# tachitachi/SR-WaveNet

Measured on AMD Instinct MI355X. Metric: audio samples/sec (fwd+bwd) 30-layer teacher WaveNet, higher is better.
Workload: dtype bf16; 1 GPU; 30-layer teacher WaveNet (3x[1..512] dilations, 64 res / 256 skip ch, 256-way mu-law softmax), fwd+bwd+Adam, batch 8x16000 samples per GPU; global_batch=8, seq_len=16000, parallelism=dp1, launch=hipGraph

## Files before the change

### sr-wavenet_amd/build.py

```python
from __future__ import annotations

import os
import subprocess
import sys
from concurrent.futures import ThreadPoolExecutor

HERE = os.path.dirname(os.path.abspath(__file__))
CSRC = os.path.join(HERE, "csrc")
LIB = os.path.join(HERE, "libsrwn.so")
MANIFEST = os.path.join(HERE, "libsrwn.manifest.json")
IO_LIB = os.path.join(HERE, "libsrwn_io.so")
PYB_SRC = os.path.join(CSRC, "srwn_pybind.cpp")
PYB_NAME = "_srwn_pyb"
IO_SOURCES = ["srwn_tfrecord.cpp"]
CXX = os.environ.get("CXX", "g++")
SOURCES = ["srwn_util.hip", "srwn_fwd.hip", "srwn_bwd.hip", "srwn_opt.hip", "srwn_pool.hip", "srwn_gemm.hip", "srwn_wgrad2.hip", "srwn_gen.hip", "srwn_gen16.hip", "srwn_flow.hip", "srwn_enc.hip", "srwn_nc.hip", "srwn_ncstream.hip", "srwn_group.hip", "srwn_wgradt.hip", "srwn_ops.hip", "srwn_head.hip", "srwn_siamese.hip", "srwn_wngate.hip", "srwn_stream.hip", "srwn_recog.hip", "srwn_score.hip"]
HIPCC = os.environ.get("HIPCC", "/opt/rocm/bin/hipcc")
FLAGS = ["--offload-arch=gfx950", "-O3", "-fPIC", "-std=c++17", "-Wno-pass-failed", "-ffp-contract=on"]
NO_SPILL = {"srwn_wgradt.hip": ["wgrad_skip_wt_kernel"], "srwn_siamese.hip": ["contrastive_head_kernel"],
            "srwn_wngate.hip": ["wavenet_layer_fwd_kernel", "wavenet_layer_bwd_kernel"],
            "srwn_ncstream.hip": ["nc_encode_frames_kernel", "nc_encode_frames_kernelINS_10NcListArgs"],
            "srwn_recog.hip": ["pooled_stream_head_kernel"], "srwn_score.hip": ["stream_score_head_kernel"]}


def _deps():
    hdrs = [os.path.join(CSRC, f) for f in os.listdir(CSRC) if f.endswith(".h")]
    hdrs.append(os.path.join(HERE, "..", "include", "srwn.h"))
    return hdrs


def source_hashes():
    import hashlib
    files = [os.path.join(CSRC, f) for f in sorted(os.listdir(CSRC)) if f.endswith((".hip", ".h", ".cpp"))]
    files.append(os.path.join(HERE, "..", "include", "srwn.h"))
    files.append(os.path.join(HERE, "..", "include", "srwn_io.h"))
    out = {}
    for f in files:
        if os.path.exists(f):
            out[os.path.relpath(f, os.path.join(HERE, ".."))] = hashlib.sha256(open(f, "rb").read()).hexdigest()
    return out


def _stale(target, srcs):
    if not os.path.exists(target):
        return True
    t = os.path.getmtime(target)
    return any(os.path.getmtime(s) > t for s in srcs)


def _sha(paths, extra=""):
    import hashlib
    h = hashlib.sha256(extra.encode())
    for f in paths:
        h.update(open(f, "rb").read())
    return h.hexdigest()


def _check_no_spill(src, obj, remarks, kernels):
    import re
    seen = {}
    name = None
    for line in remarks.splitlines():
        m = re.search(r"Function Name: (\S+)", line)
        if m:
            name = m.group(1)
        m = re.search(r"(?:[VS]GPRs Spill|ScratchSize \[bytes/lane\]): (\d+)", line)
        if m and name:
            seen[name] = seen.get(name, 0) + int(m.group(1))
    for k in kernels:
        hit = [(n, v) for n, v in seen.items() if k in n]
        if not hit or any(v for _, v in hit):
            if os.path.exists(obj):
                os.remove(obj)
            raise RuntimeError("%s: kernel %s must not spill registers or use scratch: %s" % (src, k, hit or "not found"))


def _check_inflight(src, obj, flags, kernels):
    import importlib.util
    spec = importlib.util.spec_from_file_location("_srwn_asmcheck", os.path.join(HERE, "asmcheck.py"))
    ac = importlib.util.module_from_spec(spec)
    spec.loader.exec_module(ac)
    cmd = [HIPCC] + flags + ["--cuda-device-only", "-S", src, "-o", "-"]
    r = subprocess.run(cmd, capture_output=True, text=True)
    if r.returncode != 0:
        raise RuntimeError("hipcc -S failed for %s:\n%s" % (src, r.stderr[-4000:]))
    for k in kernels:
        bad = ac.check_inflight_loads(r.stdout, k)
        if bad:
            if os.path.exists(obj):
                os.remove(obj)
            raise RuntimeError("%s: kernel %s touches the destination of a load that may still be in flight:\n  %s"
                               % (src, k, "\n  ".join(bad[:8])))


def build(force: bool = False, verbose: bool = False, diag: bool = False, variant: str = "", extra_flags=()) -> str:
    import json
    per_src = {}
    for f in list(extra_flags):
        if ".hip:" in f:
            name, fl = f.split(":", 1)
            per_src.setdefault(name, []).extend(fl.split("=", 1) if fl.startswith("-mllvm=") else [fl])
    extra_flags = [f for f in extra_flags if ".hip:" not in f]
    flags = FLAGS + (["-DSRWN_DIAG"] if diag else []) + list(extra_flags)
    if variant:
        diag = True
        odir = os.path.join(CSRC, "ab_" + variant)
        os.makedirs(os.path.join(HERE, "..", "ab"), exist_ok=True)
        lib = os.path.join(HERE, "..", "ab", "libsrwn_%s.so" % variant)
    else:
        odir = os.path.join(CSRC, "diag") if diag else CSRC
        lib = os.path.join(HERE, "libsrwn_diag.so") if diag else LIB
    os.makedirs(odir, exist_ok=True)
    man_path = os.path.join(odir, "objects.manifest.json") if diag else MANIFEST
    srcs = [os.path.join(CSRC, s) for s in SOURCES if os.path.exists(os.path.join(CSRC, s))]
    objs = [os.path.join(odir, os.path.splitext(os.path.basename(s))[0] + ".o") for s in srcs]
    deps = sorted(_deps())
    try:
        old = json.load(open(man_path)).get("objects", {})
    except (OSError, ValueError):
        old = {}
    keys = {}

    def cc(pair):
        src, obj = pair
        rel = os.path.basename(src)
        sflags = flags + per_src.get(rel, [])
        key = _sha([src] + deps, " ".join(sflags))
        if force or not os.path.exists(obj) or old.get(rel) != key:
            guarded = NO_SPILL.get(rel, [])
            cmd = [HIPCC] + sflags + (["-Rpass-analysis=kernel-resource-usage"] if guarded else []) + ["-c", src, "-o", obj]
            if verbose:
                print(" ".join(cmd), flush=True)
            r = subprocess.run(cmd, capture_output=True, text=True)
            if r.returncode != 0:
                raise RuntimeError("hipcc failed for %s:\n%s" % (src, r.stderr[-8000:]))
            if guarded:
                _check_no_spill(src, obj, r.stderr, guarded)
                _check_inflight(src, obj, sflags, guarded)
        keys[rel] = key
        return obj

    with ThreadPoolExecutor(max_workers=4) as ex:
        list(ex.map(cc, zip(srcs, objs)))
    relink = force or not os.path.exists(lib) or old != keys
    if relink:
        cmd = [HIPCC, "--offload-arch=gfx950", "-shared", "-fPIC", "-o", lib] + objs
        r = subprocess.run(cmd, capture_output=True, text=True)
        if r.returncode != 0:
            raise RuntimeError("link failed:\n%s" % r.stderr[-8000:])
    if diag:
        with open(man_path, "w") as f:
            json.dump({"flags": flags, "objects": keys}, f, indent=1, sort_keys=True)
        return lib
    build_io(force)
    build_pybind(force or relink)
    with open(MANIFEST, "w") as f:
        json.dump({"flags": flags, "objects": keys, "sources": source_hashes()}, f, indent=1, sort_keys=True)
    return lib


def _signatures():
    import importlib.util
    spec = importlib.util.spec_from_file_location("_srwn_lib_for_build", os.path.join(HERE, "_lib.py"))
    m = importlib.util.module_from_spec(spec)
    spec.loader.exec_module(m)
    return m


def pybind_source() -> str:
    import ctypes as C
    L = _signatures()
# ... 66 lines not shown
```

### sr-wavenet_amd/csrc/srwn_group.h

```cpp
#pragma once
#include <cstdint>
#include <cstdlib>
#include "srwn_common.h"

namespace srwn {
namespace grp {

constexpr int kMaxGroup = 8;
constexpr int kLdsBudget = 160 * 1024;

template <typename T> struct Raw4g;
template <> struct Raw4g<bf16_t> {
  typedef bf16x4 type;
  static __device__ __forceinline__ type load(const bf16_t* p) { return *reinterpret_cast<const bf16x4*>(p); }
  static __device__ __forceinline__ float get(const type& v, int e) { return (float)v[e]; }
  static __device__ __forceinline__ type zero() { return type{(bf16_t)0.0f, (bf16_t)0.0f, (bf16_t)0.0f, (bf16_t)0.0f}; }
  static __device__ __forceinline__ type pack(float a, float b, float c, float d) {
    return type{(bf16_t)a, (bf16_t)b, (bf16_t)c, (bf16_t)d};
  }
};
template <> struct Raw4g<float> {
  typedef f32x4 type;
  static __device__ __forceinline__ type load(const float* p) { return *reinterpret_cast<const f32x4*>(p); }
  static __device__ __forceinline__ float get(const type& v, int e) { return v[e]; }
  static __device__ __forceinline__ type zero() { return type{0.f, 0.f, 0.f, 0.f}; }
  static __device__ __forceinline__ type pack(float a, float b, float c, float d) { return type{a, b, c, d}; }
};

__device__ __forceinline__ void glds16_untracked(const void* g, unsigned lds_addr) {
  unsigned keep;
  asm volatile("s_mov_b32 %0, m0\n\ts_mov_b32 m0, %2\n\ts_nop 0\n\tglobal_load_lds_dwordx4 %1, off\n\ts_mov_b32 m0, %0"
               : "=&s"(keep) : "v"(g), "s"(lds_addr) : "memory");
}
__device__ __forceinline__ void dma_wait() { asm volatile("s_waitcnt vmcnt(0)" ::: "memory"); }
__device__ __forceinline__ void dma_image(const void* gsrc, unsigned lds_dst, int nbytes, int wave, int lane,
                                          int nwaves = 8) {
  const char* g = reinterpret_cast<const char*>(gsrc) + lane * 16;
  for (int p = wave; p < nbytes / 1024; p += nwaves) glds16_untracked(g + (size_t)p * 1024, __builtin_amdgcn_readfirstlane(lds_dst + p * 1024));
}

__device__ __forceinline__ void wg_barrier() { asm volatile("s_waitcnt lgkmcnt(0)\n\ts_barrier" ::: "memory"); }

__device__ __forceinline__ constexpr int kordW(int kg, int j) { return 16 * (kg >> 1) + 2 * (kg & 1) + (j >> 2) + 4 * (j & 3); }

template <typename T> struct LdT16;
template <> struct LdT16<bf16_t> {
  static __device__ __forceinline__ Frag<bf16_t> load(const bf16_t* tile, int stride, int row0, int col0, int lane) {
    typedef short s16x4 __attribute__((ext_vector_type(4)));
    const int kg = lane >> 4, i = lane & 15, q = i >> 2, p = i & 3;
    const bf16_t* base = tile + (size_t)(row0 + 16 * (kg >> 1) + 2 * (kg & 1) + 4 * q) * stride + col0 + 4 * p;
    s16x4 lo = __builtin_amdgcn_ds_read_tr16_b64_v4i16((__attribute__((address_space(3))) s16x4*)(base));
    s16x4 hi = __builtin_amdgcn_ds_read_tr16_b64_v4i16((__attribute__((address_space(3))) s16x4*)(base + stride));
    Frag<bf16_t> f;
    f.v = __builtin_bit_cast(bf16x8, __builtin_shufflevector(lo, hi, 0, 1, 2, 3, 4, 5, 6, 7));
    return f;
  }
};
template <> struct LdT16<float> {
  static __device__ __forceinline__ Frag<float> load(const float* tile, int stride, int row0, int col0, int lane) {
    const int kg = lane >> 4;
    const float* base = tile + (size_t)row0 * stride + col0 + (lane & 15);
    Frag<float> f;
#pragma unroll
    for (int j = 0; j < 8; ++j) f.set(j, base[(size_t)kordW(kg, j) * stride]);
// ... 138 lines not shown
```

### sr-wavenet_amd/csrc/srwn_group.hip

```cpp
#include <cmath>
#include <cstdlib>
#include <type_traits>
#include <vector>
#include "srwn_common.h"
#include "srwn_group.h"
#include "srwn_host.h"
#include "../../include/srwn.h"

using namespace srwn;
using namespace srwn::grp;

namespace {

struct GroupFwdArgs {
  int safe_wait;
  const void* x0;
  void* x_out;
  void* z_out;
  int64_t layer_stride;
  const void* wconv[kMaxGroup];
  const void* wres[kMaxGroup];
  const float* bias_f[kMaxGroup];
  const float* bias_r[kMaxGroup];
  const void* cond[kMaxGroup];
// ... 478 lines not shown
      stamp(18);
    }
  }
}

struct GroupBwdArgs {
  const void* g_top;
  void* g_out;
  void* df_out;
  const void* z;
  const void* dcs;
  int64_t layer_stride;
  const void* wconvT[kMaxGroup];
  const void* wresT[kMaxGroup];
  int sub[kMaxGroup];
  int hb[kMaxGroup];
  int nl, st, Tlen, B;
  int W, H, NT, nsub, nseg;
  const void* xT; const void* cT; int64_t wt_stride; int KT;
  void* part_f; void* part_r; float* part_bf; float* part_br;
  int nslabs, write_all_g, part16;
  const float* ic_audio; float* ic_part; int ic_shift;
  unsigned long long* stamps;
  int dbg;
};
#ifdef SRWN_DIAG
#define WT_DBG(a) ((a).dbg)
#else
#define WT_DBG(a) 0
#endif

constexpr int kWtPadRows = 64;
constexpr bool kWtEarlyR = true;
constexpr bool kWtStagger = false;
constexpr bool kWtEarlyC = false;

template <typename T, int RT, bool DCS, int MAXT, int NWB, int NWV = 8, bool WT = false, bool STAMP = false, bool P16 = false, bool ICG = false>
__global__ __launch_bounds__(64 * NWV) void group_bwd_kernel(GroupBwdArgs a) {
  static_assert(!P16 || (WT && sizeof(T) == 2), "16-bit partial blocks: the bf16 weight-gradient-tile mode only");
  static_assert(!ICG || WT, "input conv gradient: the weight-gradient-tile mode only");
  constexpr int R = 32 * RT, K = 2, KS = R / 16;
  Stamper<STAMP> stamp{nullptr, 0};
  if (STAMP && blockIdx.x == 0 && (threadIdx.x & 63) == 0 && ((threadIdx.x >> 6) & 3) == 0) stamp.p = a.stamps + (threadIdx.x >> 8) * 512;
  stamp(1);
  constexpr int NCONV = RT * K * KS, NRES = RT * KS, NW = NCONV + NRES;
  constexpr int LS = RowStage<T>::stride(R), VEC = RowStage<T>::VEC;
  constexpr int LPR = R / VEC, RPI = 64 / LPR, NI = 32 / RPI;
  constexpr int WBYTES = NW * 64 * (int)sizeof(Frag<T>);
  constexpr int WPIECES = WBYTES / 16, CPIECES = NCONV * 64 * (int)sizeof(Frag<T>) / 16;
  constexpr int KTMAX = NWV * MAXT;
  typedef typename Raw4g<T>::type raw4;
  extern __shared__ __attribute__((aligned(16))) char smem[];
  Frag<T>* wbuf = reinterpret_cast<Frag<T>*>(smem);
  T* img = reinterpret_cast<T*>(smem + (size_t)NWB * WBYTES);

  const int tid = threadIdx.x, lane = tid & 63, wave = __builtin_amdgcn_readfirstlane(tid >> 6);
  const int col = lane & 31, half = lane >> 5;
  const int rsub = lane / LPR, piece = lane % LPR;

  const unsigned lds_base = (unsigned)(size_t)(__attribute__((address_space(3))) char*)smem;
  auto wload = [&](int g, int buf) {
    dma_image(a.wconvT[g], lds_base + buf * WBYTES, CPIECES * 16, wave, lane, NWV);
    dma_image(a.wresT[g], lds_base + buf * WBYTES + CPIECES * 16, (WPIECES - CPIECES) * 16, wave, lane, NWV);
  };
  const int ntw = (a.NT - wave + NWV - 1) / NWV;

  int sit = -1;
  for (int sblk = blockIdx.x; sblk < a.nseg; sblk += gridDim.x) {
    const int seg = xcd_segment(sblk, a.nseg);
    ++sit;
    const int per_clip = a.st * a.nsub;
// ... 36 lines not shown
#pragma unroll
        for (int gq = 0; gq < 4; ++gq)
          store4(trow + (size_t)col * LS + 32 * mt + 8 * gq + 4 * half, vals[mt][4 * gq], vals[mt][4 * gq + 1],
                 vals[mt][4 * gq + 2], vals[mt][4 * gq + 3]);
      wave_lds_order();
      if (hi > 0) {
#pragma unroll
        for (int i = 0; i < NI; ++i) {
          int rr = i * RPI + rsub;
          rr = rr < hi ? rr : hi - 1;
          const f32x4 v = *reinterpret_cast<const f32x4*>(trow + (size_t)rr * LS + piece * VEC);
          *reinterpret_cast<f32x4*>(gbase + grow(jbase + 32 * q + rr) * R + piece * VEC) = v;
        }
      }
    };

    auto tile_store_raw = [&](T* trow, T* gbase, int q, int hi, const raw4 (&vals)[RT][4]) {
      wave_lds_order();
#pragma unroll
      for (int mt = 0; mt < RT; ++mt)
#pragma unroll
        for (int gq = 0; gq < 4; ++gq)
          *reinterpret_cast<raw4*>(trow + (size_t)col * LS + 32 * mt + 8 * gq + 4 * half) = vals[mt][gq];
      wave_lds_order();
#pragma unroll
      for (int i = 0; i < NI; ++i) {
        int rr = i * RPI + rsub;
        rr = rr < hi ? rr : hi - 1;
        const f32x4 v = *reinterpret_cast<const f32x4*>(trow + (size_t)rr * LS + piece * VEC);
        *reinterpret_cast<f32x4*>(gbase + grow(jbase + 32 * q + rr) * R + piece * VEC) = v;
      }
    };

    raw4 G[MAXT][RT][4];
    Frag<T> acn[8];
    const int gtop = a.nl - 1;
    auto colsum = [&](float* pb_slab, int ntiles, bool mask) {
      if (!WT || wave >= R / 16) return;
      int lw = lane;
      asm volatile("" : "+v"(lw));
      const T* cb = LdT16p<T>::base(img, LS, lw) + 16 * wave;
      Frag<T> ones;
#pragma unroll
      for (int e = 0; e < 8; ++e) ones.set(e, 1.0f);
      f32x4 accb = {0.f, 0.f, 0.f, 0.f};
      const int kfull = Wseg >> 5;
      const int nfull = mask ? (kfull < ntiles ? kfull : ntiles) : ntiles;
      constexpr int CU = 4;
#pragma unroll 1
      for (int k0 = 0; k0 < nfull; k0 += CU) {
        Frag<T> bf[CU];
#pragma unroll
        for (int u = 0; u < CU; ++u) {
          const int k = k0 + u < nfull ? k0 + u : nfull - 1;
          bf[u] = LdT16p<T>::template load<LS>(cb + (size_t)(32 * k) * LS, 0);
        }
#pragma unroll
        for (int u = 0; u < CU; ++u) {
          if (k0 + u < nfull) mma16(accb, ones, bf[u]);
        }
      }
      if (mask && nfull < ntiles) {
        const int hik = Wseg - 32 * nfull;
        Frag<T> ok;
#pragma unroll
        for (int e = 0; e < 8; ++e) ok.set(e, kordW(lw >> 4, e) < hik ? 1.0f : 0.0f);
        const Frag<T> bfl = LdT16p<T>::template load<LS>(cb + (size_t)(32 * nfull) * LS, 0);
        mma16(accb, ok, bfl);
      }
      if (lw < 16) {
        float* pb = pb_slab + 16 * wave + lw;
        *pb = (sit > 0 ? *pb : 0.0f) + accb[0];
      }
    };
    if (WT) {
      f32x4* p = reinterpret_cast<f32x4*>(img);
      for (int i = tid; i < (a.NT * 32 + kWtPadRows) * LS * (int)sizeof(T) / 16; i += 64 * NWV) p[i] = f32x4{0.f, 0.f, 0.f, 0.f};
      wg_barrier();
    }
    wload(gtop, 0);
    f32x4 zr[NI], dr[NI];
    auto issue = [&](int g, int q) {
      rows_load(reinterpret_cast<const T*>(a.z) + (size_t)g * a.layer_stride, q, zr);
      if (DCS) rows_load(reinterpret_cast<const T*>(a.dcs) + (size_t)g * a.layer_stride, q, dr);
    };
#pragma unroll
    for (int m = 0; m < MAXT; ++m) {
      const int q = wave + NWV * m;
#pragma unroll
      for (int mt = 0; mt < RT; ++mt)
#pragma unroll
        for (int gq = 0; gq < 4; ++gq) G[m][mt][gq] = Raw4g<T>::zero();
      if (q < a.NT && a.g_top) {
        T* trow = img + (size_t)(32 * q) * LS;
        f32x4 v[NI];
        rows_load(reinterpret_cast<const T*>(a.g_top), q, v);
        rows_put(trow, v);
        acc_get(trow, G[m]);
        if (WT && !((jbase + 32 * q + col) < Jr)) {
#pragma unroll
          for (int mt = 0; mt < RT; ++mt)
#pragma unroll
            for (int gq = 0; gq < 4; ++gq) G[m][mt][gq] = Raw4g<T>::zero();
        }
      }
    }
    dma_wait();
    issue(gtop, wave < a.NT ? wave : a.NT - 1);
    wg_barrier();

    for (int n = 0; n < a.nl; ++n) {
      const int g = a.nl - 1 - n;
      const int d = a.sub[g];
      int wb = 0;
      if (NWB == 2) {
        wb = n & 1;
        if (g > 0) wload(g - 1, wb ^ 1);
      } else if (n > 0) {
        wload(g, 0); dma_wait(); wg_barrier();
      }
      const Frag<T>* lds_conv = wbuf + (size_t)wb * NW * 64;
      const Frag<T>* lds_res = lds_conv + NCONV * 64;
      T* dfg = reinterpret_cast<T*>(a.df_out) + (size_t)g * a.layer_stride;
      T* gprev = reinterpret_cast<T*>(a.g_out) + (size_t)(g + 1) * a.layer_stride;
      const bool haveg = (n > 0) || (a.g_top != nullptr);
      const int hb = a.hb[g];
      int ntA = (Wseg + hb + d + 31) / 32, ntB = (Wseg + hb + 31) / 32;
      ntA = (a.H == 0 || ntA > a.NT) ? a.NT : ntA;
      ntB = (a.H == 0 || ntB > a.NT) ? a.NT : ntB;

      constexpr int NIB = R / 16, NBLK = NIB * NIB;
      constexpr int NBW = NBLK >= NWV ? NBLK / NWV : 1;
      const bool active2 = NBLK >= NWV || wave < NBLK;
      const int blk2 = wave * NBW, ib2 = blk2 / NIB, ob2 = blk2 - ib2 * NIB;
      const size_t pslab = (size_t)g * a.nslabs + blockIdx.x;
      const int ktn = (Wseg + 31) / 32;
      if (WT) {
        const bool active = active2;
        const int ib = ib2, ob0 = ob2;
        f32x4 acc[NBW];
#pragma unroll
        for (int bb = 0; bb < NBW; ++bb) acc[bb] = f32x4{0.f, 0.f, 0.f, 0.f};
        int lw = lane;
        asm volatile("" : "+v"(lw));
        if (kWtEarlyR && sizeof(T) == 2 && haveg && active && !(WT_DBG(a) & 1)) {
          const T* ct0 = reinterpret_cast<const T*>(a.cT) + (size_t)g * a.wt_stride + (size_t)seg * a.KT * (R * 32);
#pragma unroll
          for (int j = 0; j < 8; ++j) acn[j] = wt_load(ct0 + (size_t)(j < ktn ? j : (ktn > 0 ? ktn - 1 : 0)) * (R * 32), 16 * ib, lw);
        }
        if (haveg) {
#pragma unroll
          for (int m = 0; m < MAXT; ++m) {
            const int q = wave + NWV * m;
            int hi = Wseg - 32 * q;
            hi = hi > 32 ? 32 : hi;
            if (q < a.NT && hi > 0) {
              T* trow = img + (size_t)(32 * q) * LS;
              const bool own = col < hi;
              wave_lds_order();
#pragma unroll
              for (int mt = 0; mt < RT; ++mt)
#pragma unroll
                for (int gq = 0; gq < 4; ++gq)
                  *reinterpret_cast<raw4*>(trow + (size_t)col * LS + 32 * mt + 8 * gq + 4 * half) = own ? G[m][mt][gq] : Raw4g<T>::zero();
              wave_lds_order();
              if (a.write_all_g && n > 0) {
#pragma unroll
                for (int i = 0; i < NI; ++i) {
                  int rr = i * RPI + rsub;
                  rr = rr < hi ? rr : hi - 1;
                  const f32x4 v = *reinterpret_cast<const f32x4*>(trow + (size_t)rr * LS + piece * VEC);
                  *reinterpret_cast<f32x4*>(gprev + grow(jbase + 32 * q + rr) * R + piece * VEC) = v;
                }
              }
            }
          }
          stamp(20);
          wg_barrier();
          stamp(21);
          colsum(a.part_br + pslab * R, ktn, false);
          if (active && !(WT_DBG(a) & 1)) {
            const T* ct = reinterpret_cast<const T*>(a.cT) + (size_t)g * a.wt_stride + (size_t)seg * a.KT * (R * 32);
            const T* gbase = LdT16p<T>::base(img, LS, lw) + 16 * ob0;
            Frag<T> av[8], bv[8];
            if ((kWtEarlyR && sizeof(T) == 2) || (kWtEarlyC && n > 0)) {
#pragma unroll
              for (int j = 0; j < 8; ++j) av[j] = acn[j];
            } else {
#pragma unroll
              for (int j = 0; j < 8; ++j) av[j] = wt_load(ct + (size_t)(j < ktn ? j : (ktn > 0 ? ktn - 1 : 0)) * (R * 32), 16 * ib, lw);
            }
            auto group8 = [&](int k0, Frag<T> (&cur)[8], Frag<T> (&nxt)[8]) __attribute__((always_inline)) {
#pragma unroll
              for (int j = 0; j < 8; ++j) {
                const int kn = k0 + 8 + j;
                if ((WT_DBG(a) & 128) && (wave & 1)) nxt[j] = zero_frag<T>();
                else
                nxt[j] = wt_load(ct + (size_t)(kn < ktn ? kn : ktn - 1) * (R * 32), 16 * ib, lw);
              }
#pragma unroll
              for (int j = 0; j < 8; ++j) {
                const int k = k0 + j;
// ... 35 lines not shown
              }
              if (!(WT_DBG(a) & 16)) __builtin_nontemporal_store(Raw4g<bf16_t>::pack(acc[bb][0], acc[bb][1], acc[bb][2], acc[bb][3]), reinterpret_cast<p4*>(pl + bb * 256));
            }
          } else {
          float* pl = reinterpret_cast<float*>(a.part_r) + pslab * (R * R) + (size_t)(16 * ib + 4 * (lw >> 4)) * R + 16 * ob0 + (lw & 15);
          if (sit > 0) {
#pragma unroll
            for (int bb = 0; bb < NBW; ++bb) {
#pragma unroll
              for (int rr = 0; rr < 4; ++rr) acc[bb][rr] += pl[rr * R + 16 * bb];
            }
          }
#pragma unroll
          for (int bb = 0; bb < NBW; ++bb) {
            if (!(WT_DBG(a) & 16)) {
#pragma unroll
            for (int rr = 0; rr < 4; ++rr) pl[rr * R + 16 * bb] = acc[bb][rr];
            }
          }
          }
        }
        if (!haveg) colsum(a.part_br + pslab * R, 0, false);
      }

      stamp(24);
#pragma unroll
      for (int m = 0; m < MAXT; ++m) {
        const int q = wave + NWV * m;
        if (q >= ntA) continue;
        T* trow = img + (size_t)(32 * q) * LS;
        const bool ok = (jbase + 32 * q + col) < Jr;
        int hi = Wseg - 32 * q;
        hi = hi > 32 ? 32 : hi;
        if (!WT && n > 0 && hi > 0) tile_store_raw(trow, gprev, q, hi, G[m]);
        raw4 zz[RT][4], dc0[RT][4];
        rows_put(trow, zr);
        acc_get(trow, zz);
        if (DCS) { rows_put(trow, dr); acc_get(trow, dc0); }
        {
          const bool same = (m + 1 < MAXT) && (q + NWV < ntA);
          if (same) issue(g, q + NWV);
          else if (g > 0) issue(g - 1, wave < a.NT ? wave : a.NT - 1);
        }
        f32x16 accC[RT];
        if (DCS && !ok) {
#pragma unroll
          for (int mt = 0; mt < RT; ++mt)
#pragma unroll
            for (int gq = 0; gq < 4; ++gq) dc0[mt][gq] = Raw4g<T>::zero();
        }
#pragma unroll
        for (int mt = 0; mt < RT; ++mt)
#pragma unroll
          for (int gq = 0; gq < 4; ++gq)
#pragma unroll
            for (int e = 0; e < 4; ++e) accC[mt][4 * gq + e] = DCS ? Raw4g<T>::get(dc0[mt][gq], e) : 0.0f;
        if (haveg) {
#pragma unroll
          for (int s = 0; s < KS; ++s) {
            Frag<T> bfr;
            if constexpr (WT && sizeof(T) == 2) {
              bf16x4 hv[2];
#pragma unroll
              for (int h2 = 0; h2 < 2; ++h2) {
                const raw4& gr = G[m][s >> 1][2 * (s & 1) + h2];
                f32x4 g4 = {Raw4g<T>::get(gr, 0), Raw4g<T>::get(gr, 1), Raw4g<T>::get(gr, 2), Raw4g<T>::get(gr, 3)};
                g4 = g4 * f32x4{kSqrtHalf, kSqrtHalf, kSqrtHalf, kSqrtHalf};
                hv[h2] = Raw4g<bf16_t>::pack(g4[0], g4[1], g4[2], g4[3]);
              }
              bfr.v = __builtin_shufflevector(hv[0], hv[1], 0, 1, 2, 3, 4, 5, 6, 7);
            } else
#pragma unroll
            for (int jj = 0; jj < 8; ++jj)
              bfr.set(jj, ((WT || ok) ? Raw4g<T>::get(G[m][s >> 1][2 * (s & 1) + (jj >> 2)], jj & 3) : 0.0f) * kSqrtHalf);
#pragma unroll
            for (int mt = 0; mt < RT; ++mt) mma(accC[mt], lds_res[(mt * KS + s) * 64 + lane], bfr);
          }
        }
        float dv[RT][16];
        if constexpr (sizeof(T) == 2) {
#pragma unroll
          for (int mt = 0; mt < RT; ++mt)
#pragma unroll
            for (int gq = 0; gq < 4; ++gq) {
              const f32x4 z4 = {Raw4g<T>::get(zz[mt][gq], 0), Raw4g<T>::get(zz[mt][gq], 1), Raw4g<T>::get(zz[mt][gq], 2), Raw4g<T>::get(zz[mt][gq], 3)};
              const f32x4 a4 = {accC[mt][4 * gq], accC[mt][4 * gq + 1], accC[mt][4 * gq + 2], accC[mt][4 * gq + 3]};
              const f32x4 d4 = a4 * dgate_df4(z4);
#pragma unroll
              for (int e = 0; e < 4; ++e) dv[mt][4 * gq + e] = d4[e];
            }
        } else
        {
#pragma unroll
        for (int mt = 0; mt < RT; ++mt)
#pragma unroll
          for (int gq = 0; gq < 4; ++gq)
#pragma unroll
            for (int e = 0; e < 4; ++e)
              dv[mt][4 * gq + e] = accC[mt][4 * gq + e] * dgate_df<T>(Raw4g<T>::get(zz[mt][gq], e));
        }
        tile_store(trow, dfg, q, WT ? 0 : hi, dv);
        __builtin_amdgcn_sched_barrier(0);
      }
      stamp(25);
      wg_barrier();
      stamp(26);

      constexpr int NIB5 = R / 16, NBLK5 = NIB5 * NIB5;
      constexpr int NBF = 2 * NBLK5 >= NWV ? 2 * NBLK5 / NWV : 1;
      const bool active5 = WT && (2 * NBLK5 >= NWV || wave < 2 * NBLK5);
      const int blk5 = wave * NBF, tap5 = blk5 / NBLK5, rem5 = blk5 - tap5 * NBLK5, ib5 = rem5 / NIB5, ob5 = rem5 - ib5 * NIB5;
      int lw5 = lane;
      asm volatile("" : "+v"(lw5));
      const T* xt5 = reinterpret_cast<const T*>(a.xT) + (size_t)g * a.wt_stride + (size_t)seg * a.KT * (R * 32);
      if (kWtEarlyC && WT && g > 0 && active2) {
        const T* ctn = reinterpret_cast<const T*>(a.cT) + (size_t)(g - 1) * a.wt_stride + (size_t)seg * a.KT * (R * 32);
#pragma unroll
        for (int j = 0; j < 8; ++j) acn[j] = wt_load(ctn + (size_t)(j < ktn ? j : (ktn > 0 ? ktn - 1 : 0)) * (R * 32), 16 * ib2, lw5);
      }

      auto phaseB = [&]() {
#pragma unroll
      for (int m = 0; m < MAXT; ++m) {
        const int q = wave + NWV * m;
        if (q >= ntB) continue;
        const int i0 = 32 * q + col;
        const int j = jbase + i0;
        const bool ok = j < Jr;
        const bool ok_d = (j + d) < Jr;
        int src = i0 + d;
        if (!WT) src = src < a.NT * 32 ? src : a.NT * 32 - 1;
        f32x16 accG[RT];
        if constexpr (WT) {
#pragma unroll
          for (int mt = 0; mt < RT; ++mt)
#pragma unroll
            for (int gq = 0; gq < 4; ++gq) {
              f32x4 g4 = {Raw4g<T>::get(G[m][mt][gq], 0), Raw4g<T>::get(G[m][mt][gq], 1), Raw4g<T>::get(G[m][mt][gq], 2), Raw4g<T>::get(G[m][mt][gq], 3)};
              g4 = g4 * f32x4{kSqrtHalf, kSqrtHalf, kSqrtHalf, kSqrtHalf};
#pragma unroll
              for (int e = 0; e < 4; ++e) accG[mt][4 * gq + e] = g4[e];
            }
        } else
        {
#pragma unroll
        for (int mt = 0; mt < RT; ++mt)
#pragma unroll
          for (int e = 0; e < 16; ++e)
            accG[mt][e] = (haveg && (WT || ok)) ? Raw4g<T>::get(G[m][mt][e >> 2], e & 3) * kSqrtHalf : 0.0f;
        }
#pragma unroll
        for (int ks = 0; ks < KS; ++ks) {
          const Frag<T> f0 = load_nat(img + (size_t)src * LS + 16 * ks + 8 * half);
          const Frag<T> bfr = (WT || ok_d) ? f0 : zero_frag<T>();
#pragma unroll
          for (int mt = 0; mt < RT; ++mt) mma(accG[mt], lds_conv[(mt * (K * KS) + ks) * 64 + lane], bfr);
        }
#pragma unroll
        for (int ks = 0; ks < KS; ++ks) {
          const Frag<T> f1 = load_nat(img + (size_t)i0 * LS + 16 * ks + 8 * half);
          const Frag<T> bfr = (WT || ok) ? f1 : zero_frag<T>();
#pragma unroll
          for (int mt = 0; mt < RT; ++mt) mma(accG[mt], lds_conv[(mt * (K * KS) + KS + ks) * 64 + lane], bfr);
        }
#pragma unroll
        for (int mt = 0; mt < RT; ++mt)
#pragma unroll
          for (int gq = 0; gq < 4; ++gq)
            G[m][mt][gq] = Raw4g<T>::pack(accG[mt][4 * gq], accG[mt][4 * gq + 1], accG[mt][4 * gq + 2], accG[mt][4 * gq + 3]);
        __builtin_amdgcn_sched_barrier(0);
      }
      };
      auto dwf = [&]() {
        const bool active = active5;
        const int tap = tap5, ib = ib5, ob0 = ob5;
        colsum(a.part_bf + pslab * R, WT_DBG(a) & 2 ? 0 : ktn, true);
        if (active) {
          const int lw = lw5;
          const int shift = tap == 0 ? d : 0;
          f32x4 acc[NBF];
#pragma unroll
          for (int bb = 0; bb < NBF; ++bb) acc[bb] = f32x4{0.f, 0.f, 0.f, 0.f};
          const T* xt = xt5;
          const int ibl = (WT_DBG(a) & 8) ? 0 : ib;
          const int ktl = (WT_DBG(a) & 2) ? 0 : ktn;
          const T* dbase = LdT16p<T>::base(img, LS, lw) + (size_t)shift * LS + 16 * ob0;
          Frag<T> av[8], bv[8];
#pragma unroll
          for (int j = 0; j < 8; ++j) av[j] = wt_load(xt + (size_t)(j < ktn ? j : (ktn > 0 ? ktn - 1 : 0)) * (R * 32), 16 * ibl, lw);
          auto group8 = [&](int k0, Frag<T> (&cur)[8], Frag<T> (&nxt)[8]) __attribute__((always_inline)) {
#pragma unroll
            for (int j = 0; j < 8; ++j) {
              const int kn = k0 + 8 + j;
              if ((WT_DBG(a) & 128) && wave >= NWV / 2) nxt[j] = zero_frag<T>();
              else
              nxt[j] = wt_load(xt + (size_t)(kn < ktn ? kn : ktn - 1) * (R * 32), 16 * ibl, lw);
            }
#pragma unroll
            for (int j = 0; j < 8; ++j) {
              const int k = k0 + j;
              if (k < ktn) {
                const T* pk = dbase + (size_t)(32 * k) * LS;
// ... 70 lines not shown
          if ((s_ticket & 3u) == 3u) {
            __builtin_amdgcn_fence(__ATOMIC_ACQUIRE, "agent");
            const unsigned b0 = (blockIdx.x & 7u) + (blockIdx.x & ~31u);
            f32x4 sum = {0.f, 0.f, 0.f, 0.f};
            for (unsigned j = 0; j < 4; ++j) {
              const size_t slab = (size_t)g * a.nslabs + b0 + 8u * j;
              const f32x4* pf = reinterpret_cast<const f32x4*>(reinterpret_cast<const float*>(a.part_f) + slab * (2 * R * R)) + threadIdx.x;
              const f32x4* pr = reinterpret_cast<const f32x4*>(reinterpret_cast<const float*>(a.part_r) + slab * (R * R)) + threadIdx.x;
              constexpr int NF = 2 * R * R / 4 / (64 * NWV), NR = R * R / 4 / (64 * NWV);
              f32x4 v[NF + NR > 0 ? NF + NR : 1];
#pragma unroll
              for (int i = 0; i < NF; ++i) asm volatile("global_load_dwordx4 %0, %1, off sc1" : "=v"(v[i]) : "v"(pf + i * 64 * NWV) : "memory");
#pragma unroll
              for (int i = 0; i < NR; ++i) asm volatile("global_load_dwordx4 %0, %1, off sc1" : "=v"(v[NF + i]) : "v"(pr + i * 64 * NWV) : "memory");
              asm volatile("s_waitcnt vmcnt(0)" ::: "memory");
#pragma unroll
              for (int i = 0; i < NF + NR; ++i) { asm volatile("" : "+v"(v[i])); sum += v[i]; }
            }
            if (sum[0] + sum[1] + sum[2] + sum[3] == 12345.678f) counters[4095] = 1;
          }
        }
      }
#endif
      wg_barrier();
      stamp(30);
    }
#pragma unroll
    for (int m = 0; m < MAXT; ++m) {
      const int q = wave + NWV * m;
      if (q >= a.NT) continue;
      int hi = Wseg - 32 * q;
      hi = hi > 32 ? 32 : hi;
      if (hi <= 0) continue;
      tile_store_raw(img + (size_t)(32 * q) * LS, reinterpret_cast<T*>(a.g_out), q, hi, G[m]);
    }
    wg_barrier();
    if constexpr (ICG) {
      {
        constexpr int NCB = R / 16, NH = NWV / NCB;
        static_assert(NWV % NCB == 0, "waves split evenly over the column blocks");
        int lw = lane;
        asm volatile("" : "+v"(lw));
        const int cblk = wave % NCB, h = wave / NCB;
        const T* cb = LdT16p<T>::base(img, LS, lw) + 16 * cblk;
        const int arow = lw & 15, kg = lw >> 4;
        const float* au = a.ic_audio + clip;
        const int ktn = (Wseg + 31) / 32;
        const int tb = jbase * a.st + r - a.ic_shift - (arow < 2 ? 1 : 0);
        const bool tap_row = arow < 4, one_row = arow == 4;
        f32x4 acc = {0.f, 0.f, 0.f, 0.f};
#pragma unroll 4
        for (int k = h; k < ktn; k += NH) {
          Frag<T> af;
#pragma unroll
          for (int e = 0; e < 8; ++e) {
            const int pos = 32 * k + kordW(kg, e);
            const bool own = pos < Wseg;
            const int tt = tb + pos * a.st;
            const bool ld = tap_row && own && tt >= 0 && tt < a.Tlen;
            const float x = ld ? au[ld ? tt : 0] : 0.0f;
            float val;
            if (sizeof(T) == 2) {
              const float hi_ = (float)(bf16_t)x;
              val = (arow & 1) ? (x - hi_) : hi_;
            } else {
              val = (arow & 1) ? 0.0f : x;
            }
// ... 87 lines not shown
  const size_t row_bytes = (size_t)RowStage<T>::stride(R) * sizeof(T);
  const int nt_max = fwd_nt_max<T, RT, MAXT, NWB, NWV>();
  const int wmax = nt_max * 32 - a.H;
  if (wmax < 32) return set_error(SRWN_E_UNSUPPORTED, "residual_group_fwd_stream: halo %d too large", a.H);
  a.st_act = a.st < n ? a.st : n;
  const int J = (n + a.st - 1) / a.st;
  int ns = (J + wmax - 1) / wmax;
  const long long streams = (long long)a.B * a.st_act;
  long long want = (num_cus() + streams - 1) / streams;
  const int floor_w = 32 * NWV - a.H;
  long long cap = J / floor_w; if (cap < 1) cap = 1;
  if (want > cap) want = cap;
  if (want > ns) ns = (int)want;
  int w = (J + ns - 1) / ns;
  if (w < 1) w = 1;
  a.W = w;
  a.nsub = (J + w - 1) / w;
  a.NT = (a.H + w + 31) / 32;
  const long long nseg = streams * a.nsub;
  if (nseg > 0x7fffffffLL) return set_error(SRWN_E_SHAPE, "residual_group_fwd_stream: too many segments");
  a.nseg = (int)nseg;
  const size_t sh = fixed + (size_t)a.NT * 32 * row_bytes;
  const int grid_cap = group_grid();
  const long long blocks = nseg < grid_cap ? nseg : grid_cap;
  dim3 grid((unsigned)blocks), block(64 * NWV);
  auto kfn = group_fwd_kernel<T, RT, true, MAXT, NWB, NWV, true, false, false, false, true, SLOTS, ZS>;
  hipError_t e = hipFuncSetAttribute((const void*)kfn, hipFuncAttributeMaxDynamicSharedMemorySize, (int)sh);
  if (e != hipSuccess) return set_error((int)e, "residual_group_fwd_stream: LDS %zu: %s", sh, hipGetErrorString(e));
  hipLaunchKernelGGL(kfn, grid, block, sh, st, a);
  return check_launch(SLOTS ? (ZS ? "residual_group_fwd_stream_z_slots" : "residual_group_fwd_stream_slots")
                            : (ZS ? "residual_group_fwd_stream_z" : "residual_group_fwd_stream"));
}

template <typename T, int RT, int MAXT, int NWB, int NWV = 8, bool WT = false>
int launch_group_bwd(GroupBwdArgs& a, int seg_rows, hipStream_t st) {
  constexpr int R = 32 * RT, KS = R / 16, NW = RT * 2 * KS + RT * KS;
  const size_t row_bytes = (size_t)RowStage<T>::stride(R) * sizeof(T);
  const size_t fixed = (size_t)NWB * NW * 64 * sizeof(Frag<T>) + (WT ? (size_t)kWtPadRows * row_bytes : 0);
  const int nt_max = bwd_nt_max<T, RT, MAXT, NWB, NWV>(WT);
  if (nt_max * 32 - a.H < 32) return set_error(SRWN_E_UNSUPPORTED, "residual_group_bwd: halo %d too large", a.H);
  const int J = (a.Tlen + a.st - 1) / a.st;
  choose_segments(J, &a.H, a.B, a.st, nt_max, seg_rows, &a.W, &a.NT, &a.nsub);
  const long long nseg = (long long)a.B * a.st * a.nsub;
  if (nseg > 0x7fffffffLL) return set_error(SRWN_E_SHAPE, "residual_group_bwd: too many segments");
  a.nseg = (int)nseg;
  const size_t sh = fixed + (size_t)a.NT * 32 * row_bytes;
  const int grid_cap = group_grid();
  long long blocks = nseg < grid_cap ? nseg : grid_cap;
  if (WT) {
    if (a.W != seg_rows) return set_error(SRWN_E_SHAPE, "residual_group_bwd_wt: seg_rows %d does not fit (use srwn_group_wt_geometry)", seg_rows);
    a.KT = (a.W + 31) / 32;
    if (blocks > a.nslabs) return set_error(SRWN_E_SHAPE, "residual_group_bwd_wt: %lld workgroups but %d partial slabs", blocks, a.nslabs);
  }
  dim3 grid((unsigned)blocks), block(64 * NWV);
  constexpr int MT2 = MAXT > 2 ? 2 : MAXT;
  const bool two = MAXT > 2 && a.NT <= 2 * NWV;
#define SRWN_GB(D)                                                                                              \
  {                                                                                                             \
    auto kfn = two ? group_bwd_kernel<T, RT, D, MT2, NWB, NWV, WT> : group_bwd_kernel<T, RT, D, MAXT, NWB, NWV, WT>; \
    if constexpr (WT && sizeof(T) == 2) {                                                                          \
      if (a.part16) kfn = two ? group_bwd_kernel<T, RT, D, MT2, NWB, NWV, WT, false, true> : group_bwd_kernel<T, RT, D, MAXT, NWB, NWV, WT, false, true>; \
    }                                                                                                           \
    if constexpr (WT && D) {                                                                                     \
      if (a.ic_audio) {                                                                                          \
        if (a.part16) kfn = two ? group_bwd_kernel<T, RT, D, MT2, NWB, NWV, WT, false, sizeof(T) == 2, true> : group_bwd_kernel<T, RT, D, MAXT, NWB, NWV, WT, false, sizeof(T) == 2, true>; \
        else kfn = two ? group_bwd_kernel<T, RT, D, MT2, NWB, NWV, WT, false, false, true> : group_bwd_kernel<T, RT, D, MAXT, NWB, NWV, WT, false, false, true>; \
      }                                                                                                          \
    } else {                                                                                                     \
      if (a.ic_audio) return set_error(SRWN_E_UNSUPPORTED, "residual_group_bwd_wt: the input conv gradient is built for stacks with a skip path"); \
    }                                                                                                           \
    if constexpr (WT && D && sizeof(T) == 2 && RT == 2) {                                                        \
      SRWN_DIAG_ONLY(if (g_stamps && !a.part16 && !a.ic_audio) { a.stamps = g_stamps; if (!(a.dbg & 32)) kfn = two ? group_bwd_kernel<T, RT, D, MT2, NWB, NWV, WT, true> : group_bwd_kernel<T, RT, D, MAXT, NWB, NWV, WT, true>; }) \
    }                                                                                                           \
    hipError_t e = hipFuncSetAttribute((const void*)kfn, hipFuncAttributeMaxDynamicSharedMemorySize, (int)sh);  \
    if (e != hipSuccess) return set_error((int)e, "residual_group_bwd: LDS %zu: %s", sh, hipGetErrorString(e)); \
    hipLaunchKernelGGL(kfn, grid, block, sh, st, a);                                                            \
    return check_launch("residual_group_bwd");                                                                  \
  }
  if (a.dcs) SRWN_GB(true) else SRWN_GB(false)
#undef SRWN_GB
}

}

namespace {
struct WtBwd {
  const void* xT; const void* cT; int64_t wt_stride;
  void* part_f; void* part_r; float* part_bf; float* part_br; int nslabs; int write_all_g; int part16;
  const float* ic_audio; float* ic_part; int ic_shift;
};
}

static int group_bwd_impl(const void* g_top, void* g_out, void* df_out, const void* z, const void* dcs,
                          int64_t layer_stride, const void* const* wconvT, const void* const* wresT,
                          const int32_t* dilations, int32_t nlayers, int32_t B, int32_t T, int32_t R,
                          int32_t K, int32_t seg_rows, int32_t dtype, void* stream, const WtBwd* wt) {
  if (B == 0 || T == 0 || nlayers == 0) return 0;
  if (!g_out || (!df_out && !wt) || !z || !wconvT || !wresT || !dilations)
    return set_error(SRWN_E_NULL, "residual_group_bwd: null pointer");
  if (wt && (!wt->xT || !wt->cT || !wt->part_f || !wt->part_r || !wt->part_bf || !wt->part_br))
    return set_error(SRWN_E_NULL, "residual_group_bwd_wt: null pointer");
  if (wt && (seg_rows < 1 || wt->nslabs < 1 || wt->wt_stride < 0))
    return set_error(SRWN_E_SHAPE, "residual_group_bwd_wt: seg_rows=%d nslabs=%d (take them from srwn_group_wt_geometry)", seg_rows, wt->nslabs);
  if (K != 2) return set_error(SRWN_E_UNSUPPORTED, "residual_group_bwd: filter_width %d (only 2 is built)", K);
  if (R != 32 && R != 64) return set_error(SRWN_E_UNSUPPORTED, "residual_group_bwd: dilation_channels %d (built: 32, 64)", R);
  if (nlayers < 0 || nlayers > kMaxGroup || B < 0 || T < 0 || seg_rows < 0)
    return set_error(SRWN_E_SHAPE, "residual_group_bwd: nlayers=%d (max %d) B=%d T=%d", nlayers, kMaxGroup, B, T);
  if (layer_stride < (int64_t)B * T * R) return set_error(SRWN_E_SHAPE, "residual_group_bwd: layer_stride %lld", (long long)layer_stride);
  if (!g_top && !dcs) return set_error(SRWN_E_SHAPE, "residual_group_bwd: no top gradient and no skip path: every gradient would be zero");
// ... 419 lines not shown
```

Baseline: 80.05 million samples/s.

## Stage top gradient tiles via async LDS DMA and add optional LDS strip for third tile

The top-of-stack gradient tiles are now fetched straight into LDS with non-temporal global_load_lds DMA before the weight load, replacing the per-wave register load-and-put. This lets that transfer overlap with the weight and z/dcs loads. An optional STRIP variant keeps the third tile round's accumulators in an extra LDS strip instead of registers, to relieve register pressure; it is off by default. A build check also guards the affected kernels against scratch use.

Result: no change. 80.45 million samples/s (median of 6 runs) (+0.5%).

```diff
diff --git a/sr-wavenet_amd/build.py b/sr-wavenet_amd/build.py
--- a/sr-wavenet_amd/build.py
+++ b/sr-wavenet_amd/build.py
@@ -21,6 +21,7 @@
             "srwn_wngate.hip": ["wavenet_layer_fwd_kernel", "wavenet_layer_bwd_kernel"],
             "srwn_ncstream.hip": ["nc_encode_frames_kernel", "nc_encode_frames_kernelINS_10NcListArgs"],
             "srwn_recog.hip": ["pooled_stream_head_kernel"], "srwn_score.hip": ["stream_score_head_kernel"]}
+NO_SCRATCH = {"srwn_group.hip": ["group_bwd_kernelIDF16bLi2ELb%dELi%dELi2ELi8ELb1ELb0E" % (d, t) for d in (0, 1) for t in (2, 3)]}
 
 
 def _deps():
@@ -73,6 +74,24 @@
             if os.path.exists(obj):
                 os.remove(obj)
             raise RuntimeError("%s: kernel %s must not spill registers or use scratch: %s" % (src, k, hit or "not found"))
+
+
+def _check_no_scratch(src, obj, remarks, kernels):
+    import re
+    seen, name = {}, None
+    for line in remarks.splitlines():
+        m = re.search(r"Function Name: (\S+)", line)
+        if m:
+            name = m.group(1)
+        m = re.search(r"ScratchSize \[bytes/lane\]: (\d+)", line)
+        if m and name:
+            seen[name] = int(m.group(1))
+    for k in kernels:
+        hit = [(n, v) for n, v in seen.items() if k in n]
+        if not hit or any(v for _, v in hit):
+            if os.path.exists(obj):
+                os.remove(obj)
+            raise RuntimeError("%s: kernel %s must not use scratch: %s" % (src, k, [h for h in hit if h[1]] or "not found"))
 
 
 def _check_inflight(src, obj, flags, kernels):
@@ -128,7 +147,8 @@
         key = _sha([src] + deps, " ".join(sflags))
         if force or not os.path.exists(obj) or old.get(rel) != key:
             guarded = NO_SPILL.get(rel, [])
-            cmd = [HIPCC] + sflags + (["-Rpass-analysis=kernel-resource-usage"] if guarded else []) + ["-c", src, "-o", obj]
+            dry = NO_SCRATCH.get(rel, [])
+            cmd = [HIPCC] + sflags + (["-Rpass-analysis=kernel-resource-usage"] if guarded or dry else []) + ["-c", src, "-o", obj]
             if verbose:
                 print(" ".join(cmd), flush=True)
             r = subprocess.run(cmd, capture_output=True, text=True)
@@ -137,6 +157,8 @@
             if guarded:
                 _check_no_spill(src, obj, r.stderr, guarded)
                 _check_inflight(src, obj, sflags, guarded)
+            if dry:
+                _check_no_scratch(src, obj, r.stderr, dry)
         keys[rel] = key
         return obj
 
diff --git a/sr-wavenet_amd/csrc/srwn_group.h b/sr-wavenet_amd/csrc/srwn_group.h
--- a/sr-wavenet_amd/csrc/srwn_group.h
+++ b/sr-wavenet_amd/csrc/srwn_group.h
@@ -30,6 +30,11 @@
 __device__ __forceinline__ void glds16_untracked(const void* g, unsigned lds_addr) {
   unsigned keep;
   asm volatile("s_mov_b32 %0, m0\n\ts_mov_b32 m0, %2\n\ts_nop 0\n\tglobal_load_lds_dwordx4 %1, off\n\ts_mov_b32 m0, %0"
+               : "=&s"(keep) : "v"(g), "s"(lds_addr) : "memory");
+}
+__device__ __forceinline__ void glds16_untracked_nt(const void* g, unsigned lds_addr) {
+  unsigned keep;
+  asm volatile("s_mov_b32 %0, m0\n\ts_mov_b32 m0, %2\n\ts_nop 0\n\tglobal_load_lds_dwordx4 %1, off nt\n\ts_mov_b32 m0, %0"
                : "=&s"(keep) : "v"(g), "s"(lds_addr) : "memory");
 }
 __device__ __forceinline__ void dma_wait() { asm volatile("s_waitcnt vmcnt(0)" ::: "memory"); }
diff --git a/sr-wavenet_amd/csrc/srwn_group.hip b/sr-wavenet_amd/csrc/srwn_group.hip
--- a/sr-wavenet_amd/csrc/srwn_group.hip
+++ b/sr-wavenet_amd/csrc/srwn_group.hip
@@ -534,11 +534,22 @@
 
 constexpr int kWtPadRows = 64;
 constexpr bool kWtEarlyR = true;
+#ifndef SRWN_GB_TOPDMA_NT
+#define SRWN_GB_TOPDMA_NT 1
+#endif
+constexpr bool kTopDmaNt = SRWN_GB_TOPDMA_NT != 0;
+#ifndef SRWN_GB_STRIP
+#define SRWN_GB_STRIP 0
+#endif
+constexpr bool kGStrip = SRWN_GB_STRIP != 0;
 constexpr bool kWtStagger = false;
 constexpr bool kWtEarlyC = false;
 
-template <typename T, int RT, bool DCS, int MAXT, int NWB, int NWV = 8, bool WT = false, bool STAMP = false, bool P16 = false, bool ICG = false>
+template <typename T, int RT, bool DCS, int MAXT, int NWB, int NWV = 8, bool WT = false, bool STAMP = false, bool P16 = false, bool ICG = false,
+          bool STRIP = false>
 __global__ __launch_bounds__(64 * NWV) void group_bwd_kernel(GroupBwdArgs a) {
+  static_assert(!STRIP || MAXT == 3, "the strip replaces the third tile round's registers");
+  constexpr int GR = STRIP ? MAXT - 1 : MAXT;
   static_assert(!P16 || (WT && sizeof(T) == 2), "16-bit partial blocks: the bf16 weight-gradient-tile mode only");
   static_assert(!ICG || WT, "input conv gradient: the weight-gradient-tile mode only");
   constexpr int R = 32 * RT, K = 2, KS = R / 16;
@@ -641,7 +652,14 @@
       }
     };
 
-    raw4 G[MAXT][RT][4];
+    raw4 G[GR][RT][4];
+    T* gstrip = img + ((size_t)a.NT * 32 + (WT ? kWtPadRows : 0) + (size_t)wave * 32) * LS;
+    auto acc_put = [&](T* trow, const raw4 (&v)[RT][4]) {
+#pragma unroll
+      for (int mt = 0; mt < RT; ++mt)
+#pragma unroll
+        for (int gq = 0; gq < 4; ++gq) *reinterpret_cast<raw4*>(trow + (size_t)col * LS + 32 * mt + 8 * gq + 4 * half) = v[mt][gq];
+    };
     Frag<T> acn[8];
     const int gtop = a.nl - 1;
     auto colsum = [&](float* pb_slab, int ntiles, bool mask) {
@@ -687,35 +705,57 @@
       for (int i = tid; i < (a.NT * 32 + kWtPadRows) * LS * (int)sizeof(T) / 16; i += 64 * NWV) p[i] = f32x4{0.f, 0.f, 0.f, 0.f};
       wg_barrier();
     }
-    wload(gtop, 0);
     f32x4 zr[NI], dr[NI];
     auto issue = [&](int g, int q) {
       rows_load(reinterpret_cast<const T*>(a.z) + (size_t)g * a.layer_stride, q, zr);
       if (DCS) rows_load(reinterpret_cast<const T*>(a.dcs) + (size_t)g * a.layer_stride, q, dr);
     };
+    constexpr int PPR = LS * (int)sizeof(T) / 16, NPC = 32 * PPR, NDI = (NPC + 63) / 64;
+    static_assert(LS * (int)sizeof(T) % 16 == 0 && PPR == LPR + 1, "an image row is whole 16-byte pieces: its channels and one pad piece");
+    if (a.g_top) {
+      int lw = lane;
+      asm volatile("" : "+v"(lw));
+#pragma unroll
+      for (int m = 0; m < MAXT; ++m) {
+        const int q = wave + NWV * m;
+        if (q < a.NT) {
+          const unsigned dst = lds_base + NWB * WBYTES + (unsigned)(32 * q) * (LS * (int)sizeof(T));
+#pragma unroll
+          for (int u = 0; u < NDI; ++u) {
+            const int idx = u * 64 + lw;
+            if (idx < NPC) {
+              const int row = idx / PPR, pc = idx - row * PPR;
+              const T* src = reinterpret_cast<const T*>(a.g_top) + grow(jbase + 32 * q + row) * R + (pc < LPR ? pc : LPR - 1) * VEC;
+              const unsigned d = __builtin_amdgcn_readfirstlane(dst + u * 1024);
+              if (kTopDmaNt) glds16_untracked_nt(src, d); else glds16_untracked(src, d);
+            }
+          }
+        }
+      }
+    }
+    wload(gtop, 0);
+    issue(gtop, wave < a.NT ? wave : a.NT - 1);
+    dma_wait();
 #pragma unroll
     for (int m = 0; m < MAXT; ++m) {
       const int q = wave + NWV * m;
+      raw4 Gs[RT][4];
+      raw4 (&Gm)[RT][4] = (STRIP && m == GR) ? Gs : G[m < GR ? m : 0];
 #pragma unroll
       for (int mt = 0; mt < RT; ++mt)
 #pragma unroll
-        for (int gq = 0; gq < 4; ++gq) G[m][mt][gq] = Raw4g<T>::zero();
+        for (int gq = 0; gq < 4; ++gq) Gm[mt][gq] = Raw4g<T>::zero();
       if (q < a.NT && a.g_top) {
-        T* trow = img + (size_t)(32 * q) * LS;
-        f32x4 v[NI];
-        rows_load(reinterpret_cast<const T*>(a.g_top), q, v);
-        rows_put(trow, v);
-        acc_get(trow, G[m]);
+        acc_get(img + (size_t)(32 * q) * LS, Gm);
         if (WT && !((jbase + 32 * q + col) < Jr)) {
 #pragma unroll
           for (int mt = 0; mt < RT; ++mt)
 #pragma unroll
-            for (int gq = 0; gq < 4; ++gq) G[m][mt][gq] = Raw4g<T>::zero();
-        }
-      }
+            for (int gq = 0; gq < 4; ++gq) Gm[mt][gq] = Raw4g<T>::zero();
+        }
+      }
+      if (STRIP && m == GR && q < a.NT) acc_put(gstrip, Gs);
     }
-    dma_wait();
-    issue(gtop, wave < a.NT ? wave : a.NT - 1);
     wg_barrier();
 
     for (int n = 0; n < a.nl; ++n) {
@@ -766,17 +806,22 @@
             if (q < a.NT && hi > 0) {
               T* trow = img + (size_t)(32 * q) * LS;
               const bool own = col < hi;
+              raw4 Gs[RT][4];
+              raw4 (&Gm)[RT][4] = (STRIP && m == GR) ? Gs : G[m < GR ? m : 0];
+              if (STRIP && m == GR) acc_get(gstrip, Gs);
               wave_lds_order();
 #pragma unroll
               for (int mt = 0; mt < RT; ++mt)
 #pragma unroll
                 for (int gq = 0; gq < 4; ++gq)
-                  *reinterpret_cast<raw4*>(trow + (size_t)col * LS + 32 * mt + 8 * gq + 4 * half) = own ? G[m][mt][gq] : Raw4g<T>::zero();
+                  *reinterpret_cast<raw4*>(trow + (size_t)col * LS + 32 * mt + 8 * gq + 4 * half) = own ? Gm[mt][gq] : Raw4g<T>::zero();
               wave_lds_order();
               if (a.write_all_g && n > 0) {
+                int rs = rsub;
+                asm volatile("" : "+v"(rs));
 #pragma unroll
                 for (int i = 0; i < NI; ++i) {
-                  int rr = i * RPI + rsub;
+                  int rr = i * RPI + rs;
                   rr = rr < hi ? rr : hi - 1;
                   const f32x4 v = *reinterpret_cast<const f32x4*>(trow + (size_t)rr * LS + piece * VEC);
                   *reinterpret_cast<f32x4*>(gprev + grow(jbase + 32 * q + rr) * R + piece * VEC) = v;
@@ -878,7 +923,10 @@
         const bool ok = (jbase + 32 * q + col) < Jr;
         int hi = Wseg - 32 * q;
         hi = hi > 32 ? 32 : hi;
-        if (!WT && n > 0 && hi > 0) tile_store_raw(trow, gprev, q, hi, G[m]);
+        raw4 Gs[RT][4];
+        raw4 (&Gm)[RT][4] = (STRIP && m == GR) ? Gs : G[m < GR ? m : 0];
+        if (STRIP && m == GR && !WT) acc_get(gstrip, Gs);
+        if (!WT && n > 0 && hi > 0) tile_store_raw(trow, gprev, q, hi, Gm);
         raw4 zz[RT][4], dc0[RT][4];
         rows_put(trow, zr);
         acc_get(trow, zz);
@@ -905,11 +953,17 @@
 #pragma unroll
           for (int s = 0; s < KS; ++s) {
             Frag<T> bfr;
+            raw4 gw[2];
+#pragma unroll
+            for (int h2 = 0; h2 < 2; ++h2) {
+              if (STRIP && m == GR) gw[h2] = Raw4g<T>::load(gstrip + (size_t)col * LS + 32 * (s >> 1) + 8 * (2 * (s & 1) + h2) + 4 * half);
+              else gw[h2] = Gm[s >> 1][2 * (s & 1) + h2];
+            }
             if constexpr (WT && sizeof(T) == 2) {
               bf16x4 hv[2];
 #pragma unroll
               for (int h2 = 0; h2 < 2; ++h2) {
-                const raw4& gr = G[m][s >> 1][2 * (s & 1) + h2];
+                const raw4& gr = gw[h2];
                 f32x4 g4 = {Raw4g<T>::get(gr, 0), Raw4g<T>::get(gr, 1), Raw4g<T>::get(gr, 2), Raw4g<T>::get(gr, 3)};
                 g4 = g4 * f32x4{kSqrtHalf, kSqrtHalf, kSqrtHalf, kSqrtHalf};
                 hv[h2] = Raw4g<bf16_t>::pack(g4[0], g4[1], g4[2], g4[3]);
@@ -918,9 +972,10 @@
             } else
 #pragma unroll
             for (int jj = 0; jj < 8; ++jj)
-              bfr.set(jj, ((WT || ok) ? Raw4g<T>::get(G[m][s >> 1][2 * (s & 1) + (jj >> 2)], jj & 3) : 0.0f) * kSqrtHalf);
+              bfr.set(jj, ((WT || ok) ? Raw4g<T>::get(gw[jj >> 2], jj & 3) : 0.0f) * kSqrtHalf);
 #pragma unroll
             for (int mt = 0; mt < RT; ++mt) mma(accC[mt], lds_res[(mt * KS + s) * 64 + lane], bfr);
+            if (STRIP && m == GR) __builtin_amdgcn_sched_barrier(0);
           }
         }
         float dv[RT][16];
@@ -970,6 +1025,9 @@
       for (int m = 0; m < MAXT; ++m) {
         const int q = wave + NWV * m;
         if (q >= ntB) continue;
+        raw4 Gs[RT][4];
+        raw4 (&Gm)[RT][4] = (STRIP && m == GR) ? Gs : G[m < GR ? m : 0];
+        if (STRIP && m == GR) acc_get(gstrip, Gs);
         const int i0 = 32 * q + col;
         const int j = jbase + i0;
         const bool ok = j < Jr;
@@ -982,7 +1040,7 @@
           for (int mt = 0; mt < RT; ++mt)
 #pragma unroll
             for (int gq = 0; gq < 4; ++gq) {
-              f32x4 g4 = {Raw4g<T>::get(G[m][mt][gq], 0), Raw4g<T>::get(G[m][mt][gq], 1), Raw4g<T>::get(G[m][mt][gq], 2), Raw4g<T>::get(G[m][mt][gq], 3)};
+              f32x4 g4 = {Raw4g<T>::get(Gm[mt][gq], 0), Raw4g<T>::get(Gm[mt][gq], 1), Raw4g<T>::get(Gm[mt][gq], 2), Raw4g<T>::get(Gm[mt][gq], 3)};
               g4 = g4 * f32x4{kSqrtHalf, kSqrtHalf, kSqrtHalf, kSqrtHalf};
 #pragma unroll
               for (int e = 0; e < 4; ++e) accG[mt][4 * gq + e] = g4[e];
@@ -993,7 +1051,7 @@
         for (int mt = 0; mt < RT; ++mt)
 #pragma unroll
           for (int e = 0; e < 16; ++e)
-            accG[mt][e] = (haveg && (WT || ok)) ? Raw4g<T>::get(G[m][mt][e >> 2], e & 3) * kSqrtHalf : 0.0f;
+            accG[mt][e] = (haveg && (WT || ok)) ? Raw4g<T>::get(Gm[mt][e >> 2], e & 3) * kSqrtHalf : 0.0f;
         }
 #pragma unroll
         for (int ks = 0; ks < KS; ++ks) {
@@ -1013,7 +1071,8 @@
         for (int mt = 0; mt < RT; ++mt)
 #pragma unroll
           for (int gq = 0; gq < 4; ++gq)
-            G[m][mt][gq] = Raw4g<T>::pack(accG[mt][4 * gq], accG[mt][4 * gq + 1], accG[mt][4 * gq + 2], accG[mt][4 * gq + 3]);
+            Gm[mt][gq] = Raw4g<T>::pack(accG[mt][4 * gq], accG[mt][4 * gq + 1], accG[mt][4 * gq + 2], accG[mt][4 * gq + 3]);
+        if (STRIP && m == GR) acc_put(gstrip, Gs);
         __builtin_amdgcn_sched_barrier(0);
       }
       };
@@ -1150,7 +1209,10 @@
       int hi = Wseg - 32 * q;
       hi = hi > 32 ? 32 : hi;
       if (hi <= 0) continue;
-      tile_store_raw(img + (size_t)(32 * q) * LS, reinterpret_cast<T*>(a.g_out), q, hi, G[m]);
+      raw4 Gs[RT][4];
+      raw4 (&Gm)[RT][4] = (STRIP && m == GR) ? Gs : G[m < GR ? m : 0];
+      if (STRIP && m == GR) acc_get(gstrip, Gs);
+      tile_store_raw(img + (size_t)(32 * q) * LS, reinterpret_cast<T*>(a.g_out), q, hi, Gm);
     }
     wg_barrier();
     if constexpr (ICG) {
@@ -1304,6 +1366,16 @@
                             : (ZS ? "residual_group_fwd_stream_z" : "residual_group_fwd_stream"));
 }
 
+template <typename T, int RT, bool D, int MAXT, int NWB, int NWV, bool WT, bool STAMP, bool P16, bool ICG>
+auto pick_group_bwd(bool two, bool strip) -> void (*)(GroupBwdArgs) {
+  constexpr int MT2 = MAXT > 2 ? 2 : MAXT;
+  if (two) return group_bwd_kernel<T, RT, D, MT2, NWB, NWV, WT, STAMP, P16, ICG>;
+  if constexpr (MAXT == 3) {
+    if (strip) return group_bwd_kernel<T, RT, D, MAXT, NWB, NWV, WT, STAMP, P16, ICG, true>;
+  }
+  return group_bwd_kernel<T, RT, D, MAXT, NWB, NWV, WT, STAMP, P16, ICG>;
+}
+
 template <typename T, int RT, int MAXT, int NWB, int NWV = 8, bool WT = false>
 int launch_group_bwd(GroupBwdArgs& a, int seg_rows, hipStream_t st) {
   constexpr int R = 32 * RT, KS = R / 16, NW = RT * 2 * KS + RT * KS;
@@ -1325,28 +1397,30 @@
     if (blocks > a.nslabs) return set_error(SRWN_E_SHAPE, "residual_group_bwd_wt: %lld workgroups but %d partial slabs", blocks, a.nslabs);
   }
   dim3 grid((unsigned)blocks), block(64 * NWV);
-  constexpr int MT2 = MAXT > 2 ? 2 : MAXT;
   const bool two = MAXT > 2 && a.NT <= 2 * NWV;
+  const size_t strip_bytes = a.NT > 2 * NWV ? (size_t)(a.NT - 2 * NWV) * 32 * row_bytes : 0;
+  const bool strip = kGStrip && MAXT > 2 && !two && sh + strip_bytes <= (size_t)kLdsBudget;
+  const size_t shs = strip ? sh + strip_bytes : sh;
 #define SRWN_GB(D)                                                                                              \
   {                                                                                                             \
-    auto kfn = two ? group_bwd_kernel<T, RT, D, MT2, NWB, NWV, WT> : group_bwd_kernel<T, RT, D, MAXT, NWB, NWV, WT>; \
+    auto kfn = pick_group_bwd<T, RT, D, MAXT, NWB, NWV, WT, false, false, false>(two, strip);                   \
     if constexpr (WT && sizeof(T) == 2) {                                                                          \
-      if (a.part16) kfn = two ? group_bwd_kernel<T, RT, D, MT2, NWB, NWV, WT, false, true> : group_bwd_kernel<T, RT, D, MAXT, NWB, NWV, WT, false, true>; \
+      if (a.part16) kfn = pick_group_bwd<T, RT, D, MAXT, NWB, NWV, WT, false, true, false>(two, strip);          \
     }                                                                                                           \
     if constexpr (WT && D) {                                                                                     \
       if (a.ic_audio) {                                                                                          \
-        if (a.part16) kfn = two ? group_bwd_kernel<T, RT, D, MT2, NWB, NWV, WT, false, sizeof(T) == 2, true> : group_bwd_kernel<T, RT, D, MAXT, NWB, NWV, WT, false, sizeof(T) == 2, true>; \
-        else kfn = two ? group_bwd_kernel<T, RT, D, MT2, NWB, NWV, WT, false, false, true> : group_bwd_kernel<T, RT, D, MAXT, NWB, NWV, WT, false, false, true>; \
+        if (a.part16) kfn = pick_group_bwd<T, RT, D, MAXT, NWB, NWV, WT, false, sizeof(T) == 2, true>(two, strip); \
+        else kfn = pick_group_bwd<T, RT, D, MAXT, NWB, NWV, WT, false, false, true>(two, strip);                 \
       }                                                                                                          \
     } else {                                                                                                     \
       if (a.ic_audio) return set_error(SRWN_E_UNSUPPORTED, "residual_group_bwd_wt: the input conv gradient is built for stacks with a skip path"); \
     }                                                                                                           \
     if constexpr (WT && D && sizeof(T) == 2 && RT == 2) {                                                        \
-      SRWN_DIAG_ONLY(if (g_stamps && !a.part16 && !a.ic_audio) { a.stamps = g_stamps; if (!(a.dbg & 32)) kfn = two ? group_bwd_kernel<T, RT, D, MT2, NWB, NWV, WT, true> : group_bwd_kernel<T, RT, D, MAXT, NWB, NWV, WT, true>; }) \
+      SRWN_DIAG_ONLY(if (g_stamps && !a.part16 && !a.ic_audio) { a.stamps = g_stamps; if (!(a.dbg & 32)) kfn = pick_group_bwd<T, RT, D, MAXT, NWB, NWV, WT, true, false, false>(two, strip); }) \
     }                                                                                                           \
-    hipError_t e = hipFuncSetAttribute((const void*)kfn, hipFuncAttributeMaxDynamicSharedMemorySize, (int)sh);  \
-    if (e != hipSuccess) return set_error((int)e, "residual_group_bwd: LDS %zu: %s", sh, hipGetErrorString(e)); \
-    hipLaunchKernelGGL(kfn, grid, block, sh, st, a);                                                            \
+    hipError_t e = hipFuncSetAttribute((const void*)kfn, hipFuncAttributeMaxDynamicSharedMemorySize, (int)shs); \
+    if (e != hipSuccess) return set_error((int)e, "residual_group_bwd: LDS %zu: %s", shs, hipGetErrorString(e)); \
+    hipLaunchKernelGGL(kfn, grid, block, shs, st, a);                                                           \
     return check_launch("residual_group_bwd");                                                                  \
   }
   if (a.dcs) SRWN_GB(true) else SRWN_GB(false)
```
